# uthree/tinyvc

Measured on AMD Instinct MI355X. Metric: audio-samples/sec (16 kHz) end-to-end VC, higher is better.
Workload: dtype f32 (fp32 in / out / accumulate; channel contractions as two-term fp16 splits on v_mfma_f32_32x32x16_f16: 22-bit significands, three part-products per fp32 product)

## Files before the change

tinyvc_amd/csrc/filter_up24s.hip:

```cpp
#include "conv_s2.h"
#include "small_kernels.h"
#include "split_fp16.h"
#include "tvc_common.h"

namespace tvc {

typedef unsigned u32x2 __attribute__((ext_vector_type(2)));
typedef float f32x4s __attribute__((ext_vector_type(4)));

constexpr int U24S_WPE = 2;

template <int W_, int D1_, int D2_, bool SECOND_, int E_>
struct U24S {
    static constexpr int C = 24, W = W_, D1 = D1_, D2 = D2_, E = E_, H = D1_ + D2_;
    static constexpr bool SECOND = SECOND_;
    static constexpr int NWAVES = 8, NT = 64 * NWAVES;
    static constexpr int W2 = W + 2 * E;
    static constexpr int NT2 = (W2 + 31) / 32, W2r = NT2 * 32;
    static constexpr int NT1 = (W2 + 2 * D2 + 31) / 32;
    static constexpr int HP = NT1 * 32;
    static constexpr int XW = W2 + 2 * H;
    static constexpr int XP = XW;
    static constexpr int PS = W2r + 16;
    static constexpr int ITEMS = 3 * XW, XPER = (ITEMS + NT - 1) / NT;
    static constexpr int PIECES = Up24sBlob::PIECES, FL = 320;
    static constexpr int LDS_BYTES = (6 * XP + 6 * HP + PIECES * 64) * 16 + (FL + C * PS) * 4;
    static_assert(NT2 <= NWAVES, "one second-conv tile per wave");
    static_assert(XW - H >= W2, "residual columns");
    static_assert(LDS_BYTES <= 160 * 1024, "LDS");
};

struct Up24SArgs {
    const float* x;
    const uint4* cond;
    float cbw, cbb;
    float* out;
    const u32x4* img;
    int len, xf, tiles_per_utt, ntiles;
    float interp_scale;
    const float* amax_x;
    const float* amax_c;
    float* amax_y;
    RagDev rag;
};

__device__ __forceinline__ void split4(const float (&v)[4], u32x2& p1, u32x2& p2) {
#pragma unroll
    for (int j = 0; j < 2; ++j) {
        unsigned q1, q2;
        split2(v[2 * j], v[2 * j + 1], q1, q2);
        p1[j] = q1;
        p2[j] = q2;
    }
}

__device__ __forceinline__ void ld8_g8(float (&dst)[8], const float* base, unsigned byte_off) {
    const uint4* b4 = reinterpret_cast<const uint4*>(base);
    const f32x4s q0 = __builtin_bit_cast(f32x4s, ldg_so4(b4, byte_off)), q1 = __builtin_bit_cast(f32x4s, ldg_so4(b4, byte_off + 16u));
    dst[0] = q0.x; dst[1] = q0.y; dst[2] = q0.z; dst[3] = q0.w;
    dst[4] = q1.x; dst[5] = q1.y; dst[6] = q1.z; dst[7] = q1.w;
}

template <int P, int DIL>
__device__ __forceinline__ void conv24_phase(f32x16& hi, f32x16& lo, const u32x4* src, const u32x4* wt, int col, int lo_c, int hi_c, int lane) {
    const int lh = lane >> 5;
    constexpr int TAP0[5] = {0, 0, 1, 2, 2}, GRP0[5] = {0, 2, 1, 0, 2};
    constexpr int TAP1[5] = {0, 1, 1, 2, 2}, GRP1[5] = {1, 0, 2, 1, 2};
    int row[5];
#pragma unroll
    for (int s = 0; s < 5; ++s) {
        int c = col + (lh ? TAP1[s] : TAP0[s]) * DIL;
        c = c < lo_c ? lo_c : (c > hi_c ? hi_c : c);
        row[s] = (lh ? GRP1[s] : GRP0[s]) * P + c;
    }
    f16x8 af[2][2], bf[2][2];
    auto frags = [&](int s, int fb) __attribute__((always_inline)) {
#pragma unroll
        for (int p = 0; p < 2; ++p) {
            bf[fb][p] = __builtin_bit_cast(f16x8, src[p * 3 * P + row[s]]);
            af[fb][p] = __builtin_bit_cast(f16x8, wt[(s * 2 + p) * 64 + lane]);
        }
    };
    frags(0, 0);
#pragma unroll
    for (int s = 0; s < 5; ++s) {
        const int fb = s & 1;
        if (s + 1 < 5) frags(s + 1, fb ^ 1);
        __builtin_amdgcn_sched_barrier(0);
        lo = TVC_MFMA16(af[fb][1], bf[fb][0], lo);
        hi = TVC_MFMA16(af[fb][0], bf[fb][0], hi);
        lo = TVC_MFMA16(af[fb][0], bf[fb][1], lo);
        __builtin_amdgcn_sched_barrier(0);
    }
}

template <class CF, bool RAG>
__global__ __launch_bounds__(CF::NT) __attribute__((amdgpu_waves_per_eu(U24S_WPE))) void up24s_kernel(Up24SArgs a) {
    constexpr int C = CF::C, W = CF::W, D1 = CF::D1, D2 = CF::D2, H = CF::H, E = CF::E, NT = CF::NT;
    constexpr int XP = CF::XP, HP = CF::HP, PS = CF::PS, XW = CF::XW, XPER = CF::XPER;
    extern __shared__ __attribute__((aligned(16))) uint4 smem_u[];
    u32x4* Xs = reinterpret_cast<u32x4*>(smem_u);
    u32x4* Hs = Xs + 6 * XP;
    u32x4* Wt = Hs + 6 * HP;
    float* Fl = reinterpret_cast<float*>(Wt + CF::PIECES * 64);
    float* R = Fl + CF::FL;
    const int tid = threadIdx.x, lane = tid & 63, wave = tid >> 6;
    const int l31 = lane & 31, lh = lane >> 5;
    const int rs = a.len;
    const int rsl = CF::SECOND ? rs : rs / a.xf;
    int bh = 0;
    auto utt = [&](int tile) __attribute__((always_inline)) { return rag_tile<RAG>(a.rag, tile, a.tiles_per_utt, rs, bh).b; };

    for (int i = tid; i < CF::PIECES * 64 + Up24sBlob::FLOATS / 4; i += NT) Wt[i] = a.img[i];

    float xr0[XPER][8], xr1[XPER][8], lam[XPER];
    int ig8[XPER], ic[XPER];
    bool ilive[XPER];
#pragma unroll
    for (int i = 0; i < XPER; ++i) {
        const int idx = tid + i * NT;
        int g = idx / XW;
        ic[i] = idx - g * XW;
        ilive[i] = idx < CF::ITEMS;
        ig8[i] = 8 * (g > 2 ? 2 : g);
    }
    auto fetch = [&](int tile) __attribute__((always_inline)) {
        const RagTile rt = rag_tile<RAG>(a.rag, tile, a.tiles_per_utt, rs, bh);
        const int len = rt.len, lin = CF::SECOND ? len : len / a.xf;
        const int px0 = rt.tin * W - E - H;
        const uint4* xb = reinterpret_cast<const uint4*>(RAG ? a.x + 8L * (CF::SECOND ? rt.off : rt.off / a.xf) : a.x + (long)rt.b * C * rsl);
        auto ld8 = [&](float (&dst)[8], unsigned o) __attribute__((always_inline)) {
            const f32x4s q0 = __builtin_bit_cast(f32x4s, ldg_so4(xb, o)), q1 = __builtin_bit_cast(f32x4s, ldg_so4(xb, o + 16u));
            dst[0] = q0.x; dst[1] = q0.y; dst[2] = q0.z; dst[3] = q0.w;
            dst[4] = q1.x; dst[5] = q1.y; dst[6] = q1.z; dst[7] = q1.w;
        };
#pragma unroll
        for (int i = 0; i < XPER; ++i) {
            int p = px0 + ic[i];
            p = p < 0 ? 0 : (p > len - 1 ? len - 1 : p);
            const int g = ig8[i] >> 3;
            if (CF::SECOND) {
                ld8(xr0[i], 32u * (unsigned)(g * rsl + p));
            } else {
                const Lerp lc = lerp_coord(p, a.interp_scale, lin);
                lam[i] = lc.w1;
                ld8(xr0[i], 32u * (unsigned)(g * rsl + lc.i0));
                ld8(xr1[i], 32u * (unsigned)(g * rsl + lc.i1));
            }
        }
    };
    auto deposit = [&](float xs) __attribute__((always_inline)) {
#pragma unroll
        for (int i = 0; i < XPER; ++i) {
            if (!ilive[i]) continue;
            const int g = ig8[i] >> 3, c = ic[i];
            float v[8];
            if (CF::SECOND) {
#pragma unroll
                for (int j = 0; j < 8; ++j) v[j] = xr0[i][j];
            } else {
                const float w0 = 1.f - lam[i];
#pragma unroll
                for (int j = 0; j < 8; ++j) v[j] = fmaf(w0, xr0[i][j], __fmul_rn(lam[i], xr1[i][j]));
            }
            const int rc = c - H;
            if (rc >= 0 && rc < CF::W2r) {
#pragma unroll
                for (int j = 0; j < 8; ++j) R[(ig8[i] + j) * PS + rc] = v[j];
            }
#pragma unroll
            for (int j = 0; j < 8; ++j) v[j] = fmaxf(v[j], 0.1f * v[j]) * xs;
            uint4 p1, p2;
            split8(v, p1, p2);
            Xs[(0 + g) * XP + c] = __builtin_bit_cast(u32x4, p1);
            Xs[(3 + g) * XP + c] = __builtin_bit_cast(u32x4, p2);
        }
    };

    int tile, tend;
    tile_range(a.ntiles, tile, tend);
    if (tile < tend) {
        bh = utt(tile);
        fetch(tile);
        deposit(bfp_load_u(a.amax_x, bh).s);
    }
    slab_barrier();
    const float wsa = Fl[Up24sBlob::SA], wsb = Fl[Up24sBlob::SB], wssc = Fl[Up24sBlob::SSC], wssh = Fl[Up24sBlob::SSH], wl1 = Fl[Up24sBlob::L1A], bamax = Fl[Up24sBlob::BMA];
    float mx_run = 0.f;
    int mx_b = bh;
    int slot_b = -1;
    Bfp sx{1.f, 1.f}, sc{1.f, 1.f}, sh_{1.f, 1.f};

    for (; tile < tend; ++tile) {
        const RagTile rt = rag_tile<RAG>(a.rag, tile, a.tiles_per_utt, rs, bh);
        const int b = rt.b, len = rt.len;
        bh = b;
        if (!CF::SECOND && a.amax_y && b != mx_b) {
            amax_flush_wg(a.amax_y + mx_b, mx_run, Fl + Up24sBlob::FLOATS);
            mx_run = 0.f;
            mx_b = b;
        }
        if (b != slot_b) {
            slot_b = b;
            const float slot_x = a.amax_x ? sload_f32(a.amax_x + b) : 0.f;
            const float slot_c = a.amax_c ? sload_f32(a.amax_c + b) : 0.f;
            sx = a.amax_x ? bfp_from_amax(slot_x) : Bfp{1.f, 1.f};
            sc = a.amax_c ? norm_from_amax(fmaf(a.cbw, slot_c, a.cbb)) : Bfp{1.f, 1.f};
            sh_ = a.amax_x ? bfp_from_amax(fmaf(wl1, slot_x, bamax)) : Bfp{1.f, 1.f};
        }
        const int t0 = rt.tin * W;
        const int ph0 = t0 - E - D2;
        const int p20 = t0 - E;
        const int next = tile + 1;

        float keep[3][4];
        bool keep_live = false;
        unsigned keep_oo = 0;
        float wv_out = 0.f;
        bool wv_live = false;
        int wv_off = 0;
        u32x4 cq[2][2];
        if (wave < CF::NT2) {
            const uint4* cb = RAG ? a.cond + rt.off : a.cond + (long)b * 6 * rs;
            int t = p20 + wave * 32 + l31;
            t = t < 0 ? 0 : (t > len - 1 ? len - 1 : t);
            const unsigned o0 = 16u * (unsigned)(lh * rs + t), o1 = 16u * (unsigned)t;
#pragma unroll
            for (int p = 0; p < 2; ++p) {
                cq[0][p] = ldg_so4(cb + (long)(3 * p) * rs, o0);
                cq[1][p] = ldg_so4(cb + (long)(3 * p + 2) * rs, o1);
            }
        }

        bool fetched = false;
        for (int nt = wave; nt < CF::NT1; nt += CF::NWAVES) {
            f32x16 acc, alo;
#pragma unroll
            for (int r = 0; r < 16; ++r) acc[r] = alo[r] = 0.f;
            const int h = nt * 32 + l31;
            conv24_phase<XP, D1>(acc, alo, Xs, Wt, h, 0, XW - 1, lane);
            if (!fetched) {
                fetched = true;
                if (next < tend) fetch(next);
            }
            const float c = wsa * sx.inv, cl = c * kLoInv;
#pragma unroll
            for (int g = 0; g < 3; ++g) {
                const f32x4s bv = *reinterpret_cast<const f32x4s*>(Fl + Up24sBlob::BA + 8 * g + 4 * lh);
                float v[4];
#pragma unroll
                for (int q = 0; q < 4; ++q) {
                    const float t = comb(acc[4 * g + q], alo[4 * g + q], c, cl) + bv[q];
                    v[q] = fmaxf(t, 0.1f * t) * sh_.s;
                }
                u32x2 p1, p2;
                split4(v, p1, p2);
                const auto qx = __builtin_amdgcn_permlane32_swap(p1[0], p2[0], false, false);
                const auto qy = __builtin_amdgcn_permlane32_swap(p1[1], p2[1], false, false);
                const u32x4 row = {qx[0], qy[0], qx[1], qy[1]};
                *reinterpret_cast<u32x4*>(Hs + (3 * lh + g) * HP + h) = row;
            }
        }
        if (!fetched && next < tend) fetch(next);
        slab_barrier();

        if (wave < CF::NT2) {
            const int n = wave * 32 + l31;
            const int t = p20 + n;
            f16x8 cf[2][2];
            {
                const u32x4 z = {0u, 0u, 0u, 0u};
#pragma unroll
                for (int p = 0; p < 2; ++p) {
                    cf[0][p] = __builtin_bit_cast(f16x8, cq[0][p]);
                    cf[1][p] = __builtin_bit_cast(f16x8, lh ? z : cq[1][p]);
                }
            }
            const float cb = wsb * sh_.inv, cbl = cb * kLoInv, c1 = wssc * sc.inv, c1l = c1 * kLoInv, c2 = wssh * sc.inv, c2l = c2 * kLoInv;
            float hv[3][4];
            {
                f32x16 acc, alo;
#pragma unroll
                for (int r = 0; r < 16; ++r) acc[r] = alo[r] = 0.f;
                const int lo = -ph0 > 0 ? -ph0 : 0;
                const int hi = (len - 1 - ph0) < (HP - 1) ? (len - 1 - ph0) : (HP - 1);
                conv24_phase<HP, D2>(acc, alo, Hs, Wt + 10 * 64, n, lo, hi, lane);
#pragma unroll
                for (int g = 0; g < 3; ++g) {
                    const f32x4s bb = *reinterpret_cast<const f32x4s*>(Fl + Up24sBlob::BB + 8 * g + 4 * lh);
#pragma unroll
                    for (int q = 0; q < 4; ++q) hv[g][q] = comb(acc[4 * g + q], alo[4 * g + q], cb, cbl) + bb[q];
                }
            }
            __builtin_amdgcn_sched_barrier(0);
            f32x16 asc, lsc, ash, lsh;
#pragma unroll
            for (int r = 0; r < 16; ++r) asc[r] = lsc[r] = ash[r] = lsh[r] = 0.f;
#pragma unroll
            for (int s = 0; s < 2; ++s) {
                f16x8 fa[2][2];
#pragma unroll
                for (int mt = 0; mt < 2; ++mt)
#pragma unroll
                    for (int p = 0; p < 2; ++p) fa[mt][p] = __builtin_bit_cast(f16x8, Wt[(20 + (s * 2 + mt) * 2 + p) * 64 + lane]);
                lsc = TVC_MFMA16(fa[0][1], cf[s][0], lsc);
                lsh = TVC_MFMA16(fa[1][1], cf[s][0], lsh);
                asc = TVC_MFMA16(fa[0][0], cf[s][0], asc);
                ash = TVC_MFMA16(fa[1][0], cf[s][0], ash);
                lsc = TVC_MFMA16(fa[0][0], cf[s][1], lsc);
                lsh = TVC_MFMA16(fa[1][0], cf[s][1], lsh);
            }
            float mx = 0.f;
#pragma unroll
            for (int g = 0; g < 3; ++g) {
                float v4[4];
                const f32x4s bs = *reinterpret_cast<const f32x4s*>(Fl + Up24sBlob::BSC + 8 * g + 4 * lh);
                const f32x4s bh = *reinterpret_cast<const f32x4s*>(Fl + Up24sBlob::BSH + 8 * g + 4 * lh);
#pragma unroll
                for (int q = 0; q < 4; ++q) {
                    const int m = 8 * g + 4 * lh + q;
                    const float hval = hv[g][q];
                    const float scv = comb(asc[4 * g + q], lsc[4 * g + q], c1, c1l) + bs[q];
                    const float shv = comb(ash[4 * g + q], lsh[4 * g + q], c2, c2l) + bh[q];
                    const float res = R[m * PS + n];
                    const float v = __fadd_rn(__fadd_rn(__fmul_rn(hval, scv), shv), res);
                    v4[q] = v;
                    if (CF::SECOND) R[m * PS + n] = v;
                }
                if (!CF::SECOND) {
#pragma unroll
                    for (int q = 0; q < 4; ++q) keep[g][q] = v4[q];
                    if (n < W && t < len) mx = fmaxf(mx, fmaxf(fmaxf(fabsf(v4[0]), fabsf(v4[1])), fmaxf(fabsf(v4[2]), fabsf(v4[3]))));
                }
            }
            mx_run = fmaxf(mx_run, mx);
            keep_live = !CF::SECOND && n < W && t < len;
            keep_oo = 32u * (unsigned)t + 16u * (unsigned)lh;
        }
        if (CF::SECOND) {
            slab_barrier();
            const float* W7 = Fl + Up24sBlob::W75;
            const int part = tid & 7;
            const int lo = -p20 > 0 ? -p20 : 0;
            const int hi = (len - 1 - p20) < (CF::W2 - 1) ? (len - 1 - p20) : (CF::W2 - 1);
            const bool interior = lo == 0 && hi == CF::W2 - 1;
            for (int g0 = 0; g0 < (W + 3) / 4; g0 += NT / 8) {
                const int g = g0 + (tid >> 3);
                float o4[4] = {0.f, 0.f, 0.f, 0.f};
                if (4 * g < W) {
#pragma unroll
                    for (int cc = 0; cc < 3; ++cc) {
                        const int c = part * 3 + cc;
                        float xv[10], wv[7];
                        if (E == 3 && interior) {
                            const f32x4s* rp = reinterpret_cast<const f32x4s*>(R + c * PS + 4 * g);
                            const f32x4s r0 = rp[0], r1 = rp[1], r2 = rp[2];
                            xv[0] = r0[0]; xv[1] = r0[1]; xv[2] = r0[2]; xv[3] = r0[3];
                            xv[4] = r1[0]; xv[5] = r1[1]; xv[6] = r1[2]; xv[7] = r1[3];
                            xv[8] = r2[0]; xv[9] = r2[1];
                        } else {
#pragma unroll
                            for (int i = 0; i < 10; ++i) {
                                int col = 4 * g + E - 3 + i;
                                col = col < lo ? lo : (col > hi ? hi : col);
                                xv[i] = R[c * PS + col];
                            }
                        }
#pragma unroll
                        for (int j = 0; j < 7; ++j) wv[j] = W7[c * 7 + j];
#pragma unroll
                        for (int q = 0; q < 4; ++q)
#pragma unroll
                            for (int j = 0; j < 7; ++j) o4[q] = fmaf(wv[j], xv[q + j], o4[q]);
                    }
                }
#pragma unroll
                for (int q = 0; q < 4; ++q) {
                    o4[q] += __shfl_xor(o4[q], 1);
                    o4[q] += __shfl_xor(o4[q], 2);
                    o4[q] += __shfl_xor(o4[q], 4);
                }
                const int o = 4 * g + part;
                const float v = part == 0 ? o4[0] : (part == 1 ? o4[1] : (part == 2 ? o4[2] : o4[3]));
                static_assert((W + 3) / 4 <= NT / 8, "one output per thread: it waits in a register until the deposit is through");
                wv_out = v + Fl[Up24sBlob::B75];
                wv_live = part < 4 && o < W && t0 + o < len;
                wv_off = t0 + o;
            }
        }
        slab_barrier();
        if (next < tend) {
            const int bn = utt(next);
            deposit(bn == slot_b ? sx.s : bfp_load_u(a.amax_x, bn).s);
        }
        if (CF::SECOND) {
            float* wrow = RAG ? a.out + (long)a.rag.row[b] * a.rag.Tmax * kHop : a.out + (long)b * rs;
            if (wv_live) wrow[wv_off] = wv_out;
        } else if (keep_live) {
            float* ob = RAG ? a.out + 8L * rt.off : a.out + (long)b * C * rs;
#pragma unroll
            for (int g = 0; g < 3; ++g) stg_so4(ob + (long)g * 8 * rs, keep_oo, keep[g]);
        }
        slab_barrier();
    }
    if (!CF::SECOND && a.amax_y && tend > (int)((long)a.ntiles * blockIdx.x / gridDim.x)) amax_flush_wg(a.amax_y + mx_b, mx_run, Fl + Up24sBlob::FLOATS);
}

template <class CF>
static int launch_up24s(tvc_ctx* ctx, hipStream_t s, Up24SArgs a, int B) {
    const size_t lds = (size_t)CF::LDS_BYTES;
    TVC_CHECK((lds_optin<up24s_kernel<CF, false>, up24s_kernel<CF, true>>(ctx, (int)lds, "up24s")));
    a.tiles_per_utt = (a.len + CF::W - 1) / CF::W;
    a.ntiles = a.tiles_per_utt * B;
    TVC_CHECK(rag_tiles(ctx, s, B, a.len, CF::W, &a.rag, &a.ntiles, "up24s", kHop));
    const int grid = a.ntiles < ctx->ncu ? a.ntiles : ctx->ncu;
    if (ctx->rag) hipLaunchKernelGGL((up24s_kernel<CF, true>), dim3(grid), dim3(CF::NT), lds, s, a);
    else hipLaunchKernelGGL((up24s_kernel<CF, false>), dim3(grid), dim3(CF::NT), lds, s, a);
    return launch_check(ctx, "up24s");
}

constexpr int U24S_WA = 250, U24S_WB = 250;

int run_up24_split(tvc_ctx* ctx, hipStream_t s, const UpW& u, const float* x, const float* cond_planes, float cbw, float cbb, float* x1, float* wave, int B, int len,
                   const float* amax_x, const float* amax_c, float* amax_x1) {
    if (!u.s24a || !u.s24b) return fail(ctx, TVC_ERR_STATE, "up24s: the split weight blobs of the 24-channel block are missing");
    if ((long)len * 24 * 4 >= (1L << 32)) return fail(ctx, TVC_ERR_ARG, "up24s: utterance too long for 32-bit element offsets");
    using CA = U24S<U24S_WA, 1, 3, false, 0>;
    using CB = U24S<U24S_WB, 9, 27, true, 3>;
    Up24SArgs a{};
    a.len = len;
    a.xf = u.factor;
    a.interp_scale = (float)(1.0 / (double)u.factor);
    a.cond = reinterpret_cast<const uint4*>(cond_planes);
    a.cbw = cbw;
    a.cbb = cbb;
    a.amax_c = amax_c;
    a.x = x;
    a.amax_x = amax_x;
    a.out = x1;
    a.amax_y = amax_x1;
    a.img = reinterpret_cast<const u32x4*>(u.s24a);
    TVC_CHECK(launch_up24s<CA>(ctx, s, a, B));
    a.x = x1;
    a.amax_x = amax_x1;
    a.out = wave;
    a.amax_y = nullptr;
    a.img = reinterpret_cast<const u32x4*>(u.s24b);
    return launch_up24s<CB>(ctx, s, a, B);
}

struct Down0SArgs {
    const float* source;
    const float* energy;
    float* out;
    uint4* planes;
    float* y2;
    const u32x4* img;
    int len, tiles_per_utt, ntiles;
    const float* amax_x;
    float* amax_y;
    RagDev rag;
};

template <bool RAG>
static __global__ __launch_bounds__(512) __attribute__((amdgpu_waves_per_eu(4))) void down0s_kernel(Down0SArgs a) {
    constexpr int W = 254, XW = 256, XP = XW, NT = 512;
    extern __shared__ __attribute__((aligned(16))) uint4 smem_d[];
    u32x4* Xs = reinterpret_cast<u32x4*>(smem_d);
    u32x4* Wt = Xs + 2 * 6 * XP;
    float* Bi = reinterpret_cast<float*>(Wt + Down0sBlob::PIECES * 64);
    const int tid = threadIdx.x, lane = tid & 63, wave = tid >> 6;
    const int l31 = lane & 31, lh = lane >> 5;
    const int rs = a.len;
    for (int i = tid; i < Down0sBlob::PIECES * 64 + Down0sBlob::FLOATS / 4; i += NT) Wt[i] = a.img[i];

    const int g = tid >> 8, c = tid & 255;
    float xa[8], xe = 0.f;
// ... 421 lines not shown
```

tinyvc_amd/csrc/pack.hip:

```cpp
#include <algorithm>
#include <cmath>

#include "tvc_common.h"

namespace tvc {

size_t ArenaBuilder::put(const float** slot, const float* v, size_t n) {
    const size_t off = (buf.size() + 63) & ~size_t(63);
    buf.resize(off + n, 0.f);
    std::copy(v, v + n, buf.begin() + off);
    fix.push_back({slot, off});
    return off;
}

namespace {

int pad_m(int M) {
    if (M <= 32) return 32;
    if (M <= 64) return 64;
    if (M <= 96) return 96;
    if (M % 96 == 0 && M % 128 != 0) return M;
    return (M + 127) / 128 * 128;
}

// ... 163 lines not shown
        a6(pb, Ab, 0, sa);
        ab.fix.push_back({&pb->wjoint, off_a});
    }
    size_t a6(PackedW* pw, const std::vector<float>& At, int group_rows, const std::vector<float>& scale) {
        const int taps = pw->taps, cin = pw->cin, nslab = ((cin + 15) / 16 + 5) / 6 * 6;
        const int MT = image_mt(pw, group_rows);
        std::vector<float> img((size_t)nslab * taps * MT * 2 * 256, 0.f);
        uint16_t* o = reinterpret_cast<uint16_t*>(img.data());
        for (int s = 0; s < nslab; ++s)
            for (int tap = 0; tap < taps; ++tap)
                for (int mt = 0; mt < MT; ++mt)
                    for (int lane = 0; lane < 64; ++lane)
                        for (int j = 0; j < 8; ++j) {
                            const int ci = s * 16 + 8 * (lane >> 5) + j, m = image_row(pw, group_rows, mt * 32 + (lane & 31));
                            const float w = (ci < cin && m < pw->M) ? At[(size_t)(ci * taps + tap) * pw->Mpad + m] : 0.f;
                            const size_t base = (((size_t)(s * taps + tap) * MT + mt) * 2 * 64 + lane) * 8 + j;
                            split2(w, scale[mt], &o[base], &o[base + 512]);
                        }
        pw->MT6 = MT;
        pw->S6 = nslab;
        const size_t off = ab.put(&pw->A6, img);
        ab.put(&pw->wscale, scale);
        host_wscale[pw] = scale;
        return off;
    }
    void film_u(FilmU* fu, const std::string& conv_name, const std::string& film, int C, const std::string& first_conv) {
        const size_t CC = (size_t)C * C;
        const float* w = get(conv_name + ".weight", 3 * CC);
        const float* b = get(conv_name + ".bias", C);
        const float* wsc = get(film + ".to_scale.weight", CC);
        const float* bsc = get(film + ".to_scale.bias", C);
        const float* wsh = get(film + ".to_shift.weight", CC);
        const float* bsh = get(film + ".to_shift.bias", C);
        if (!w || !b || !wsc || !bsc || !wsh || !bsh) return;
        const int MT = C / 32, nslab = C / 16, mblocks = C / 96;
        auto tile_scale = [&](const float* wt, int per_row, int mt) { return pow2_scale(amax(wt + (size_t)mt * 32 * per_row, (size_t)32 * per_row)) * (1.f / 8192.f); };
        std::vector<float> tab((size_t)6 * C);
        auto row = [&](int r) { return &tab[(size_t)r * C]; };
        float *scale_conv = row(FilmU::TAB_SCALE), *scale_sc = row(FilmU::TAB_SSC), *scale_sh = row(FilmU::TAB_SSH);
        std::copy(b, b + C, row(FilmU::TAB_BIAS));
        std::copy(bsc, bsc + C, row(FilmU::TAB_BSC));
        std::copy(bsh, bsh + C, row(FilmU::TAB_BSH));
        for (int mt = 0; mt < MT; ++mt) {
            std::fill_n(scale_conv + 32 * mt, 32, tile_scale(w, 3 * C, mt));
            std::fill_n(scale_sc + 32 * mt, 32, tile_scale(wsc, C, mt));
            std::fill_n(scale_sh + 32 * mt, 32, tile_scale(wsh, C, mt));
        }
        std::vector<float> img((size_t)mblocks * nslab * 30 * 64 * 4, 0.f);
        uint16_t* o = reinterpret_cast<uint16_t*>(img.data());
        for (int mb = 0; mb < mblocks; ++mb)
            for (int s = 0; s < nslab; ++s)
                for (int q = 0; q < 30; ++q) {
                    const bool conv = q < 18;
                    const int qq = conv ? q : q - 18, grp = qq / 6, mi = (qq % 6) / 2, part = qq % 2, mt = mb * 3 + mi;
                    for (int lane = 0; lane < 64; ++lane)
                        for (int j = 0; j < 8; ++j) {
                            const int m = mt * 32 + (lane & 31), ci = s * 16 + 8 * (lane >> 5) + j;
                            float x;
                            if (conv) x = w[((size_t)m * C + ci) * 3 + grp] / scale_conv[m];
                            else if (grp == 0) x = wsc[(size_t)m * C + ci] / scale_sc[m];
                            else x = wsh[(size_t)m * C + ci] / scale_sh[m];
                            const uint16_t h1 = f16_bits(x);
                            o[((((size_t)mb * nslab + s) * 30 + q) * 64 + lane) * 8 + j] = part == 0 ? h1 : f16_bits(x - f16_value(h1));
                        }
                }
        bound(first_conv, C, 3 * C, &fu->hb_w, &fu->hb_b);
        fu->C = C;
        ab.put(&fu->img, img);
        ab.put(&fu->tab, tab);
    }
    void up24s_half(const float** slot, const std::string& ca, const std::string& cb, const std::string& film, const std::string& c5,
                    const std::string& out7) {
        using L = Up24sBlob;
        constexpr int C = 24;
        const float* wa = get(ca + ".weight", C * C * 3);
        const float* ba = get(ca + ".bias", C);
        const float* wb = get(cb + ".weight", C * C * 3);
        const float* bb = get(cb + ".bias", C);
        const float* wsc = get(film + ".to_scale.weight", C * C);
        const float* bsc = get(film + ".to_scale.bias", C);
        const float* wsh = get(film + ".to_shift.weight", C * C);
        const float* bsh = get(film + ".to_shift.bias", C);
        if (!wa || !ba || !wb || !bb || !wsc || !bsc || !wsh || !bsh) return;
        std::vector<float> img(L::PIECES * 256 + L::FLOATS, 0.f);
        float* fl = img.data() + L::PIECES * 256;
        fl[L::SA] = pow2_scale(amax(wa, C * C * 3));
        fl[L::SB] = pow2_scale(amax(wb, C * C * 3));
        fl[L::SSC] = pow2_scale(amax(wsc, C * C));
        fl[L::SSH] = pow2_scale(amax(wsh, C * C));
        put_k24(img, 0, 2, wa, C, C, 3, &fl[L::SA]);
        put_k24(img, 10, 2, wb, C, C, 3, &fl[L::SB]);
        put_k24(img, 20, 4, wsc, C, C, 1, &fl[L::SSC]);
        put_k24(img, 22, 4, wsh, C, C, 1, &fl[L::SSH]);
        std::copy(ba, ba + C, fl + L::BA);
        std::copy(bb, bb + C, fl + L::BB);
        std::copy(bsc, bsc + C, fl + L::BSC);
        std::copy(bsh, bsh + C, fl + L::BSH);
        const RowL1 r = row_l1(wa, ba, C, C * 3);
        fl[L::L1A] = (float)(r.w * 1.0000002);
        fl[L::BMA] = (float)r.b;
        if (!c5.empty()) {
            const float* w5 = get(c5 + ".weight", C * C);
            const float* b5 = get(c5 + ".bias", C);
            const float* w7 = get(out7 + ".weight", C * 7);
            const float* b7 = get(out7 + ".bias", 1);
            if (!w5 || !b5 || !w7 || !b7) return;
            double bias = b7[0];
            for (int c = 0; c < C; ++c)
                for (int j = 0; j < 7; ++j) {
                    double acc = 0.0;
                    for (int m = 0; m < C; ++m) acc += (double)w7[(size_t)m * 7 + j] * (double)w5[(size_t)m * C + c];
                    fl[L::W75 + c * 7 + j] = (float)acc;
                }
            for (int m = 0; m < C; ++m)
                for (int j = 0; j < 7; ++j) bias += (double)w7[(size_t)m * 7 + j] * (double)b5[m];
            fl[L::B75] = (float)bias;
        }
        ab.put(slot, img);
    }
    void down0s(const float** slot, const std::string& name, float* bound_w, float* bound_b) {
        using L = Down0sBlob;
        constexpr int C = 24, CI = 17;
        const float* w = get(name + ".weight", C * CI * 3);
        const float* b = get(name + ".bias", C);
        if (!w || !b) return;
        std::vector<float> img(L::PIECES * 256 + L::FLOATS, 0.f);
        float* fl = img.data() + L::PIECES * 256;
        fl[L::SCALE] = pow2_scale(amax(w, C * CI * 3));
        put_k24(img, 0, 2, w, C, CI, 3, &fl[L::SCALE]);
        std::copy(b, b + C, fl + L::BIAS);
        const RowL1 r = row_l1(w, b, C, CI * 3);
        fl[L::BW] = *bound_w = (float)(r.w * 1.0001);
        fl[L::BB] = *bound_b = (float)r.b * 1.0001f;
        ab.put(slot, img);
    }
    void conv24s(const float** slot, const std::string& name, int M, const std::string& extra_bias = "", const PackedW* joint = nullptr) {
        constexpr int CI = 24;
        const int MT = (M + 31) / 32;
        const float* w = get(name + ".weight", (size_t)M * CI * 3);
        const float* b = get(name + ".bias", M);
        const float* eb = extra_bias.empty() ? nullptr : get(extra_bias, M);
        if (!w || !b || (!extra_bias.empty() && !eb)) return;
        std::vector<float> img((size_t)K24_PIECES * MT * 256 + Conv24sBlob::FLOATS, 0.f);
        float* fl = img.data() + (size_t)K24_PIECES * MT * 256;
        float* sc = fl + Conv24sBlob::SCALE;
        if (joint) {
            auto it = host_wscale.find(joint);
            if (it == host_wscale.end() || (int)it->second.size() != MT) return note(name + " (its joint image is not packed yet)");
            std::copy(it->second.begin(), it->second.end(), sc);
        } else {
            for (int mt = 0; mt < MT; ++mt) sc[mt] = pow2_scale(amax(w + (size_t)32 * mt * CI * 3, (size_t)(std::min(M, 32 * mt + 32) - 32 * mt) * CI * 3));
        }
        put_k24(img, 0, 2 * MT, w, M, CI, 3, sc);
        for (int m = 0; m < M; ++m) fl[Conv24sBlob::BIAS + m] = b[m] + (eb ? eb[m] : 0.f);
        ab.put(slot, img);
    }
    void convnext(const std::string& p, ConvNeXtW* w, int C, int dil) {
        w->C = C;
        w->dilation = dil;
        raw(p + ".c1.weight", &w->dw_w, (size_t)C * 7);
        raw(p + ".c1.bias", &w->dw_b, C);
        const float* g = get(p + ".norm.gamma", C);
        const float* bt = get(p + ".norm.beta", C);
        if (g) ab.put(&w->ln_g, g, C);
        if (bt) ab.put(&w->ln_b, bt, C);
        if (g && bt) {
            const RowL1 r = row_l1(g, bt, C, 1);
            w->ln_bound = std::sqrt((float)C) * (float)r.w + (float)r.b;
        }
        conv({p + ".c2"}, &w->c2, C, 1);
        raw(p + ".grn.gamma", &w->grn_g, 2 * C);
        raw(p + ".grn.beta", &w->grn_b, 2 * C);
        conv({p + ".c3"}, &w->c3, 2 * C, 1);
        const float* w3 = get(p + ".c3.weight", (size_t)C * 2 * C);
        const float* b3 = get(p + ".c3.bias", C);
        const float* gb = get(p + ".grn.beta", 2 * C);
        if (w3 && b3 && gb) {
            std::vector<float> fb(w->c3.Mpad, 0.f);
            for (int m = 0; m < C; ++m) {
                double acc = b3[m];
                for (int k = 0; k < 2 * C; ++k) acc += (double)w3[(size_t)m * 2 * C + k] * (double)gb[k];
                fb[m] = (float)acc;
            }
            ab.put(&w->c3_bias_grn, fb);
        }
    }
};

}

void pack_constants(tvc_ctx* ctx, ArenaBuilder* ab) {
    const int N = kNfft;
    const double two_pi = 6.283185307179586476925286766559;
    std::vector<float> t960(2 * 960), t1920(2 * 961 + 2), hann(N);
    for (int j = 0; j < 960; ++j) {
        t960[2 * j] = (float)std::cos(two_pi * j / 960.0);
        t960[2 * j + 1] = (float)std::sin(two_pi * j / 960.0);
    }
    for (int k = 0; k <= 960; ++k) {
// ... 111 lines not shown
```

tinyvc_amd/csrc/tvc_common.h:

```cpp
#pragma once
#include <hip/hip_runtime.h>

#include <atomic>
#include <cstdarg>
#include <cstdint>
#include <cstdio>
#include <cstring>
#include <map>
#include <string>
#include <vector>

#include "../../include/tinyvc_hip.h"
#include "ragged.h"

namespace tvc {

constexpr int kSampleRate = 24000;
constexpr int kNfft = 1920;
constexpr int kHop = 480;
constexpr int kBins = 961;
constexpr int kSslDim = 768;
constexpr int kSslCh = 384;
constexpr int kPitchCh = 128;
constexpr int kPitchClasses = 512;
constexpr int kSrcCh = 128;
constexpr int kHarm = 15;
constexpr int kSolaCross = 1920, kSolaSearch = 1920, kSolaDelay = 3840;
constexpr int kSolaGroups = 8, kSolaPartFloats = 16384;

struct PackedW {
    const float* bias = nullptr;
    const float* A6 = nullptr;
    const float* wscale = nullptr;
    const float* wjoint = nullptr;
    int M = 0, K = 0, Mpad = 0, Kpad = 0, cin = 0, taps = 1, MT6 = 0, S6 = 0;
};

struct ConvNeXtW {
    const float* dw_w = nullptr;
    const float* dw_b = nullptr;
    const float* ln_g = nullptr;
    const float* ln_b = nullptr;
    PackedW c2, c3;
    const float* grn_g = nullptr;
    const float* grn_b = nullptr;
    const float* c3_bias_grn = nullptr;
    float ln_bound = 0.f;
    int C = 0, dilation = 1;
};

constexpr int K24_PIECES = 10;
struct Up24sBlob {
    static constexpr int PIECES = 28;
    static constexpr int BA = 0, BB = 32, BSC = 64, BSH = 96;
    static constexpr int W75 = 128, B75 = 296;
    static constexpr int SA = 297, SB = 298, SSC = 299, SSH = 300;
    static constexpr int L1A = 301, BMA = 302;
    static constexpr int FLOATS = 304;
};
struct Down0sBlob {
    static constexpr int PIECES = K24_PIECES;
    static constexpr int BIAS = 0;
    static constexpr int BW = 29, BB = 30;
    static constexpr int SCALE = 31;
    static constexpr int FLOATS = 32;
};
struct Conv24sBlob {
    static constexpr int BIAS = 0;
    static constexpr int SCALE = 62;
    static constexpr int FLOATS = 64;
};

struct DownW {
    PackedW res, c1, c2, c3;
    const float* c3res_bias = nullptr;
    const float* s24c1 = nullptr;
    const float* s24c2 = nullptr;
    const float* s24c3r = nullptr;
    float b1_w = 0.f, b1_b = 0.f, b2_w = 0.f, b2_b = 0.f;
    int cin = 0, cout = 0, factor = 1;
};
struct FilmU {
    static constexpr int TAB_BIAS = 0, TAB_SCALE = 1, TAB_BSC = 2, TAB_BSH = 3, TAB_SSC = 4, TAB_SSH = 5;
    const float* img = nullptr;
    const float* tab = nullptr;
    int C = 0;
    float hb_w = 0.f, hb_b = 0.f;
};
struct UpW {
    PackedW c1, c2, c3, c4, c5, film1, film2;
    FilmU fu1, fu2;
    const float* s24a = nullptr;
    const float* s24b = nullptr;
    float c5_bw = 0.f, c5_bb = 0.f;
    int cin = 0, cout = 0, factor = 1;
};

struct HostTensor {
    std::vector<float> data;
    std::vector<int64_t> shape;
};

struct ArenaBuilder {
    std::vector<float> buf;
    std::vector<std::pair<const float**, size_t>> fix;
    size_t put(const float** slot, const float* v, size_t n);
    size_t put(const float** slot, const std::vector<float>& v) { return put(slot, v.data(), v.size()); }
    void resolve(const float* arena) const {
        for (auto& f : fix) *f.first = arena + f.second;
    }
};

}

struct tvc_prof_region {
    std::string name;
    hipEvent_t a = nullptr, b = nullptr;
};

struct tvc_ctx {
    int device = 0;
    int ncu = 0;
    int profiling = 0;
    std::vector<tvc_prof_region> regions;
    std::vector<hipEvent_t> event_pool;
    hipStream_t side = nullptr;
    hipEvent_t ev_fork = nullptr, ev_join = nullptr;
    hipEvent_t ev_fork2 = nullptr, ev_join2 = nullptr, ev_amps = nullptr;
    tvc::RagHost* rag = nullptr;
    int rag_batch_frames = 0;
    bool enc_ready = false, dec_ready = false;
    char enc_missing[160] = {0}, dec_missing[160] = {0};
    std::map<std::string, tvc::HostTensor> host;
    std::vector<float> pitch_table;
    float* arena = nullptr;
    float* const_arena = nullptr;
    size_t arena_floats = 0;
    char err[512] = {0};

    const float* fft_tw960 = nullptr;
// ... 230 lines not shown
```

Measured before the change: 718.5 million.

## Slide up24s window as LDS ring and fold final 7-tap conv into MFMA

In the second up24s stage, consecutive tiles of the same utterance now reuse the overlapping halo columns of the input, hidden and residual LDS buffers as ring buffers. Only the new W columns are fetched and only the new hidden columns are recomputed, instead of reloading and recomputing the whole window. The fused 1x1+7-tap output convolution moves from a per-thread scalar FMA loop over the residual buffer to an in-register MFMA contraction (24→7 channels) stored into a small Y buffer, followed by a 7-term diagonal sum. This adds ring-index wrapping, extra LDS and a new fp16-split packed weight, and changes rounding in the output head.

```diff
diff --git a/tinyvc_amd/csrc/filter_up24s.hip b/tinyvc_amd/csrc/filter_up24s.hip
--- a/tinyvc_amd/csrc/filter_up24s.hip
+++ b/tinyvc_amd/csrc/filter_up24s.hip
@@ -21,10 +21,17 @@
     static constexpr int HP = NT1 * 32;
     static constexpr int XW = W2 + 2 * H;
     static constexpr int XP = XW;
+    static constexpr bool RING = SECOND;
+    static constexpr int SX0 = XW - W;
+    static constexpr int SH0 = W2 + 2 * D2 - NWAVES * 32;
     static constexpr int PS = W2r + 16;
+    static constexpr int YS = W2r + 8;
     static constexpr int ITEMS = 3 * XW, XPER = (ITEMS + NT - 1) / NT;
-    static constexpr int PIECES = Up24sBlob::PIECES, FL = 320;
-    static constexpr int LDS_BYTES = (6 * XP + 6 * HP + PIECES * 64) * 16 + (FL + C * PS) * 4;
+    static constexpr int PIECES = SECOND ? Up24sBlob::PIECES2 : Up24sBlob::PIECES, FL = 320;
+    static constexpr int RW = RING ? XW - H : W2r, RS = RING ? 304 : PS;
+    static constexpr int LDS_BYTES = (6 * XP + 6 * HP + PIECES * 64) * 16 + (FL + C * RS + (SECOND ? 7 * YS : 0)) * 4;
+    static_assert(!RING || (SH0 >= 0 && SH0 <= W2 + 2 * D2 - W && SH0 + NWAVES * 32 - 1 + 2 * D1 < XW), "the slide's first-conv round covers the new Hs columns from Xs columns of this window");
+    static_assert(!RING || (HP >= W2 + 2 * D2 && RS >= RW && SX0 >= H && W <= XP && W <= HP && W <= RS), "ring capacities");
     static_assert(NT2 <= NWAVES, "one second-conv tile per wave");
     static_assert(XW - H >= W2, "residual columns");
     static_assert(LDS_BYTES <= 160 * 1024, "LDS");
@@ -61,8 +68,13 @@
     dst[4] = q1.x; dst[5] = q1.y; dst[6] = q1.z; dst[7] = q1.w;
 }
 
-template <int P, int DIL>
-__device__ __forceinline__ void conv24_phase(f32x16& hi, f32x16& lo, const u32x4* src, const u32x4* wt, int col, int lo_c, int hi_c, int lane) {
+__device__ __forceinline__ int ring_wrap(int i, int cap) {
+    const unsigned u = (unsigned)i, w = u - (unsigned)cap;
+    return (int)(u < w ? u : w);
+}
+
+template <int P, int DIL, bool RING = false>
+__device__ __forceinline__ void conv24_phase(f32x16& hi, f32x16& lo, const u32x4* src, const u32x4* wt, int col, int lo_c, int hi_c, int lane, int org = 0) {
     const int lh = lane >> 5;
     constexpr int TAP0[5] = {0, 0, 1, 2, 2}, GRP0[5] = {0, 2, 1, 0, 2};
     constexpr int TAP1[5] = {0, 1, 1, 2, 2}, GRP1[5] = {1, 0, 2, 1, 2};
@@ -71,6 +83,7 @@
     for (int s = 0; s < 5; ++s) {
         int c = col + (lh ? TAP1[s] : TAP0[s]) * DIL;
         c = c < lo_c ? lo_c : (c > hi_c ? hi_c : c);
+        if (RING) c = ring_wrap(c + org, P);
         row[s] = (lh ? GRP1[s] : GRP0[s]) * P + c;
     }
     f16x8 af[2][2], bf[2][2];
@@ -97,13 +110,15 @@
 template <class CF, bool RAG>
 __global__ __launch_bounds__(CF::NT) __attribute__((amdgpu_waves_per_eu(U24S_WPE))) void up24s_kernel(Up24SArgs a) {
     constexpr int C = CF::C, W = CF::W, D1 = CF::D1, D2 = CF::D2, H = CF::H, E = CF::E, NT = CF::NT;
-    constexpr int XP = CF::XP, HP = CF::HP, PS = CF::PS, XW = CF::XW, XPER = CF::XPER;
+    constexpr int XP = CF::XP, HP = CF::HP, PS = CF::PS, RS = CF::RS, XW = CF::XW, XPER = CF::XPER;
+    constexpr bool RING = CF::RING;
     extern __shared__ __attribute__((aligned(16))) uint4 smem_u[];
     u32x4* Xs = reinterpret_cast<u32x4*>(smem_u);
     u32x4* Hs = Xs + 6 * XP;
     u32x4* Wt = Hs + 6 * HP;
     float* Fl = reinterpret_cast<float*>(Wt + CF::PIECES * 64);
     float* R = Fl + CF::FL;
+    float* Y = R + C * RS;
     const int tid = threadIdx.x, lane = tid & 63, wave = tid >> 6;
     const int l31 = lane & 31, lh = lane >> 5;
     const int rs = a.len;
@@ -124,7 +139,19 @@
         ilive[i] = idx < CF::ITEMS;
         ig8[i] = 8 * (g > 2 ? 2 : g);
     }
-    auto fetch = [&](int tile) __attribute__((always_inline)) {
+    int sg8[XPER], sc_[XPER];
+    bool slive[XPER];
+    if (RING) {
+#pragma unroll
+        for (int i = 0; i < XPER; ++i) {
+            const int idx = tid + i * NT;
+            int g = idx / W;
+            sc_[i] = CF::SX0 + idx - g * W;
+            slive[i] = idx < 3 * W;
+            sg8[i] = 8 * (g > 2 ? 2 : g);
+        }
+    }
+    auto fetch = [&](int tile, bool slide) __attribute__((always_inline)) {
         const RagTile rt = rag_tile<RAG>(a.rag, tile, a.tiles_per_utt, rs, bh);
         const int len = rt.len, lin = CF::SECOND ? len : len / a.xf;
         const int px0 = rt.tin * W - E - H;
@@ -136,9 +163,9 @@
         };
 #pragma unroll
         for (int i = 0; i < XPER; ++i) {
-            int p = px0 + ic[i];
+            int p = px0 + (RING && slide ? sc_[i] : ic[i]);
             p = p < 0 ? 0 : (p > len - 1 ? len - 1 : p);
-            const int g = ig8[i] >> 3;
+            const int g = (RING && slide ? sg8[i] : ig8[i]) >> 3;
             if (CF::SECOND) {
                 ld8(xr0[i], 32u * (unsigned)(g * rsl + p));
             } else {
@@ -149,11 +176,11 @@
             }
         }
     };
-    auto deposit = [&](float xs) __attribute__((always_inline)) {
+    auto deposit = [&](float xs, bool slide, int ox, int orr) __attribute__((always_inline)) {
 #pragma unroll
         for (int i = 0; i < XPER; ++i) {
-            if (!ilive[i]) continue;
-            const int g = ig8[i] >> 3, c = ic[i];
+            if (!(RING && slide ? slive[i] : ilive[i])) continue;
+            const int g8 = RING && slide ? sg8[i] : ig8[i], g = g8 >> 3, c = RING && slide ? sc_[i] : ic[i];
             float v[8];
             if (CF::SECOND) {
 #pragma unroll
@@ -164,16 +191,18 @@
                 for (int j = 0; j < 8; ++j) v[j] = fmaf(w0, xr0[i][j], __fmul_rn(lam[i], xr1[i][j]));
             }
             const int rc = c - H;
-            if (rc >= 0 && rc < CF::W2r) {
-#pragma unroll
-                for (int j = 0; j < 8; ++j) R[(ig8[i] + j) * PS + rc] = v[j];
+            if (rc >= 0 && rc < CF::RW) {
+                const int rr = RING ? ring_wrap(orr + rc, RS) : rc;
+#pragma unroll
+                for (int j = 0; j < 8; ++j) R[(g8 + j) * RS + rr] = v[j];
             }
 #pragma unroll
             for (int j = 0; j < 8; ++j) v[j] = fmaxf(v[j], 0.1f * v[j]) * xs;
             uint4 p1, p2;
             split8(v, p1, p2);
-            Xs[(0 + g) * XP + c] = __builtin_bit_cast(u32x4, p1);
-            Xs[(3 + g) * XP + c] = __builtin_bit_cast(u32x4, p2);
+            const int cx = RING ? ring_wrap(ox + c, XP) : c;
+            Xs[(0 + g) * XP + cx] = __builtin_bit_cast(u32x4, p1);
+            Xs[(3 + g) * XP + cx] = __builtin_bit_cast(u32x4, p2);
         }
     };
 
@@ -181,8 +210,8 @@
     tile_range(a.ntiles, tile, tend);
     if (tile < tend) {
         bh = utt(tile);
-        fetch(tile);
-        deposit(bfp_load_u(a.amax_x, bh).s);
+        fetch(tile, false);
+        deposit(bfp_load_u(a.amax_x, bh).s, false, 0, 0);
     }
     slab_barrier();
     const float wsa = Fl[Up24sBlob::SA], wsb = Fl[Up24sBlob::SB], wssc = Fl[Up24sBlob::SSC], wssh = Fl[Up24sBlob::SSH], wl1 = Fl[Up24sBlob::L1A], bamax = Fl[Up24sBlob::BMA];
@@ -190,6 +219,8 @@
     int mx_b = bh;
     int slot_b = -1;
     Bfp sx{1.f, 1.f}, sc{1.f, 1.f}, sh_{1.f, 1.f};
+    bool slid = false;
+    int ox = 0, oh = 0, orr = 0;
 
     for (; tile < tend; ++tile) {
         const RagTile rt = rag_tile<RAG>(a.rag, tile, a.tiles_per_utt, rs, bh);
@@ -212,6 +243,8 @@
         const int ph0 = t0 - E - D2;
         const int p20 = t0 - E;
         const int next = tile + 1;
+        const int bn = next < tend ? utt(next) : -1;
+        const bool slide_next = RING && bn == b;
 
         float keep[3][4];
         bool keep_live = false;
@@ -233,15 +266,16 @@
         }
 
         bool fetched = false;
-        for (int nt = wave; nt < CF::NT1; nt += CF::NWAVES) {
+        const int nt1 = RING && slid ? CF::NWAVES : CF::NT1, h0 = RING && slid ? CF::SH0 : 0;
+        for (int nt = wave; nt < nt1; nt += CF::NWAVES) {
             f32x16 acc, alo;
 #pragma unroll
             for (int r = 0; r < 16; ++r) acc[r] = alo[r] = 0.f;
-            const int h = nt * 32 + l31;
-            conv24_phase<XP, D1>(acc, alo, Xs, Wt, h, 0, XW - 1, lane);
+            const int h = h0 + nt * 32 + l31;
+            conv24_phase<XP, D1, RING>(acc, alo, Xs, Wt, h, 0, XW - 1, lane, ox);
             if (!fetched) {
                 fetched = true;
-                if (next < tend) fetch(next);
+                if (next < tend) fetch(next, slide_next);
             }
             const float c = wsa * sx.inv, cl = c * kLoInv;
 #pragma unroll
@@ -258,10 +292,10 @@
                 const auto qx = __builtin_amdgcn_permlane32_swap(p1[0], p2[0], false, false);
                 const auto qy = __builtin_amdgcn_permlane32_swap(p1[1], p2[1], false, false);
                 const u32x4 row = {qx[0], qy[0], qx[1], qy[1]};
-                *reinterpret_cast<u32x4*>(Hs + (3 * lh + g) * HP + h) = row;
-            }
-        }
-        if (!fetched && next < tend) fetch(next);
+                *reinterpret_cast<u32x4*>(Hs + (3 * lh + g) * HP + (RING ? ring_wrap(oh + h, HP) : h)) = row;
+            }
+        }
+        if (!fetched && next < tend) fetch(next, slide_next);
         slab_barrier();
 
         if (wave < CF::NT2) {
@@ -284,7 +318,7 @@
                 for (int r = 0; r < 16; ++r) acc[r] = alo[r] = 0.f;
                 const int lo = -ph0 > 0 ? -ph0 : 0;
                 const int hi = (len - 1 - ph0) < (HP - 1) ? (len - 1 - ph0) : (HP - 1);
-                conv24_phase<HP, D2>(acc, alo, Hs, Wt + 10 * 64, n, lo, hi, lane);
+                conv24_phase<HP, D2, RING>(acc, alo, Hs, Wt + 10 * 64, n, lo, hi, lane, oh);
 #pragma unroll
                 for (int g = 0; g < 3; ++g) {
                     const f32x4s bb = *reinterpret_cast<const f32x4s*>(Fl + Up24sBlob::BB + 8 * g + 4 * lh);
@@ -311,6 +345,7 @@
                 lsh = TVC_MFMA16(fa[1][0], cf[s][1], lsh);
             }
             float mx = 0.f;
+            const int nr = RING ? ring_wrap(orr + n, RS) : n;
 #pragma unroll
             for (int g = 0; g < 3; ++g) {
                 float v4[4];
@@ -322,10 +357,13 @@
                     const float hval = hv[g][q];
                     const float scv = comb(asc[4 * g + q], lsc[4 * g + q], c1, c1l) + bs[q];
                     const float shv = comb(ash[4 * g + q], lsh[4 * g + q], c2, c2l) + bh[q];
-                    const float res = R[m * PS + n];
+                    const float res = R[m * RS + nr];
                     const float v = __fadd_rn(__fadd_rn(__fmul_rn(hval, scv), shv), res);
                     v4[q] = v;
-                    if (CF::SECOND) R[m * PS + n] = v;
+                }
+                if (CF::SECOND) {
+#pragma unroll
+                    for (int q = 0; q < 4; ++q) keep[g][q] = v4[q];
                 }
                 if (!CF::SECOND) {
 #pragma unroll
@@ -336,63 +374,70 @@
             mx_run = fmaxf(mx_run, mx);
             keep_live = !CF::SECOND && n < W && t < len;
             keep_oo = 32u * (unsigned)t + 16u * (unsigned)lh;
+            if (CF::SECOND) {
+                __builtin_amdgcn_sched_barrier(0);
+                float m2 = 0.f;
+#pragma unroll
+                for (int g = 0; g < 3; ++g)
+#pragma unroll
+                    for (int q = 0; q < 4; ++q) m2 = fmaxf(m2, fabsf(keep[g][q]));
+                const Bfp s2 = bfp_from_amax(wave_max(m2));
+                u32x2 p[2][3];
+#pragma unroll
+                for (int g = 0; g < 3; ++g) {
+                    const float v[4] = {keep[g][0] * s2.s, keep[g][1] * s2.s, keep[g][2] * s2.s, keep[g][3] * s2.s};
+                    split4(v, p[0][g], p[1][g]);
+                }
+                f16x8 xf[2][2];
+#pragma unroll
+                for (int pt = 0; pt < 2; ++pt) {
+                    const auto e0 = __builtin_amdgcn_permlane32_swap(p[pt][0][0], p[pt][1][0], false, false);
+                    const auto e1 = __builtin_amdgcn_permlane32_swap(p[pt][0][1], p[pt][1][1], false, false);
+                    const auto f0 = __builtin_amdgcn_permlane32_swap(p[pt][2][0], 0u, false, false);
+                    const auto f1 = __builtin_amdgcn_permlane32_swap(p[pt][2][1], 0u, false, false);
+                    xf[0][pt] = __builtin_bit_cast(f16x8, u32x4{e0[0], e1[0], e0[1], e1[1]});
+                    xf[1][pt] = __builtin_bit_cast(f16x8, u32x4{f0[0], f1[0], f0[1], f1[1]});
+                }
+                f32x16 yh, yl;
+#pragma unroll
+                for (int r = 0; r < 16; ++r) yh[r] = yl[r] = 0.f;
+#pragma unroll
+                for (int s = 0; s < 2; ++s) {
+                    const f16x8 w1 = __builtin_bit_cast(f16x8, Wt[(Up24sBlob::P75 + 2 * s) * 64 + lane]), w2 = __builtin_bit_cast(f16x8, Wt[(Up24sBlob::P75 + 2 * s + 1) * 64 + lane]);
+                    yl = TVC_MFMA16(w2, xf[s][0], yl);
+                    yh = TVC_MFMA16(w1, xf[s][0], yh);
+                    yl = TVC_MFMA16(w1, xf[s][1], yl);
+                }
+                const float c7 = Fl[Up24sBlob::S75] * s2.inv, c7l = c7 * kLoInv;
+#pragma unroll
+                for (int q = 0; q < 4; ++q)
+                    if (4 * lh + q < 7) Y[(4 * lh + q) * CF::YS + n] = comb(yh[q], yl[q], c7, c7l);
+            }
         }
         if (CF::SECOND) {
             slab_barrier();
-            const float* W7 = Fl + Up24sBlob::W75;
-            const int part = tid & 7;
             const int lo = -p20 > 0 ? -p20 : 0;
             const int hi = (len - 1 - p20) < (CF::W2 - 1) ? (len - 1 - p20) : (CF::W2 - 1);
-            const bool interior = lo == 0 && hi == CF::W2 - 1;
-            for (int g0 = 0; g0 < (W + 3) / 4; g0 += NT / 8) {
-                const int g = g0 + (tid >> 3);
-                float o4[4] = {0.f, 0.f, 0.f, 0.f};
-                if (4 * g < W) {
-#pragma unroll
-                    for (int cc = 0; cc < 3; ++cc) {
-                        const int c = part * 3 + cc;
-                        float xv[10], wv[7];
-                        if (E == 3 && interior) {
-                            const f32x4s* rp = reinterpret_cast<const f32x4s*>(R + c * PS + 4 * g);
-                            const f32x4s r0 = rp[0], r1 = rp[1], r2 = rp[2];
-                            xv[0] = r0[0]; xv[1] = r0[1]; xv[2] = r0[2]; xv[3] = r0[3];
-                            xv[4] = r1[0]; xv[5] = r1[1]; xv[6] = r1[2]; xv[7] = r1[3];
-                            xv[8] = r2[0]; xv[9] = r2[1];
-                        } else {
-#pragma unroll
-                            for (int i = 0; i < 10; ++i) {
-                                int col = 4 * g + E - 3 + i;
-                                col = col < lo ? lo : (col > hi ? hi : col);
-                                xv[i] = R[c * PS + col];
-                            }
-                        }
-#pragma unroll
-                        for (int j = 0; j < 7; ++j) wv[j] = W7[c * 7 + j];
-#pragma unroll
-                        for (int q = 0; q < 4; ++q)
-#pragma unroll
-                            for (int j = 0; j < 7; ++j) o4[q] = fmaf(wv[j], xv[q + j], o4[q]);
-                    }
-                }
-#pragma unroll
-                for (int q = 0; q < 4; ++q) {
-                    o4[q] += __shfl_xor(o4[q], 1);
-                    o4[q] += __shfl_xor(o4[q], 2);
-                    o4[q] += __shfl_xor(o4[q], 4);
-                }
-                const int o = 4 * g + part;
-                const float v = part == 0 ? o4[0] : (part == 1 ? o4[1] : (part == 2 ? o4[2] : o4[3]));
-                static_assert((W + 3) / 4 <= NT / 8, "one output per thread: it waits in a register until the deposit is through");
-                wv_out = v + Fl[Up24sBlob::B75];
-                wv_live = part < 4 && o < W && t0 + o < len;
-                wv_off = t0 + o;
-            }
+            static_assert(W <= NT, "one output per thread: it waits in a register until the deposit is through");
+            float acc = Fl[Up24sBlob::B75];
+#pragma unroll
+            for (int j = 0; j < 7; ++j) {
+                int col = tid + j + E - 3;
+                col = col < lo ? lo : (col > hi ? hi : col);
+                acc = __fadd_rn(acc, Y[j * CF::YS + col]);
+            }
+            wv_out = acc;
+            wv_live = tid < W && t0 + tid < len;
+            wv_off = t0 + tid;
         }
         slab_barrier();
-        if (next < tend) {
-            const int bn = utt(next);
-            deposit(bn == slot_b ? sx.s : bfp_load_u(a.amax_x, bn).s);
-        }
+        if (RING) {
+            ox = slide_next ? ring_wrap(ox + W, XP) : 0;
+            oh = slide_next ? ring_wrap(oh + W, HP) : 0;
+            orr = slide_next ? ring_wrap(orr + W, RS) : 0;
+            slid = slide_next;
+        }
+        if (next < tend) deposit(bn == slot_b ? sx.s : bfp_load_u(a.amax_x, bn).s, slide_next, ox, orr);
         if (CF::SECOND) {
             float* wrow = RAG ? a.out + (long)a.rag.row[b] * a.rag.Tmax * kHop : a.out + (long)b * rs;
             if (wv_live) wrow[wv_off] = wv_out;
diff --git a/tinyvc_amd/csrc/pack.hip b/tinyvc_amd/csrc/pack.hip
--- a/tinyvc_amd/csrc/pack.hip
+++ b/tinyvc_amd/csrc/pack.hip
@@ -269,8 +269,9 @@
         const float* wsh = get(film + ".to_shift.weight", C * C);
         const float* bsh = get(film + ".to_shift.bias", C);
         if (!wa || !ba || !wb || !bb || !wsc || !bsc || !wsh || !bsh) return;
-        std::vector<float> img(L::PIECES * 256 + L::FLOATS, 0.f);
-        float* fl = img.data() + L::PIECES * 256;
+        const int pieces = c5.empty() ? L::PIECES : L::PIECES2;
+        std::vector<float> img(pieces * 256 + L::FLOATS, 0.f);
+        float* fl = img.data() + pieces * 256;
         fl[L::SA] = pow2_scale(amax(wa, C * C * 3));
         fl[L::SB] = pow2_scale(amax(wb, C * C * 3));
         fl[L::SSC] = pow2_scale(amax(wsc, C * C));
@@ -302,6 +303,11 @@
             for (int m = 0; m < C; ++m)
                 for (int j = 0; j < 7; ++j) bias += (double)w7[(size_t)m * 7 + j] * (double)b5[m];
             fl[L::B75] = (float)bias;
+            float w75t[7 * C];
+            for (int c = 0; c < C; ++c)
+                for (int j = 0; j < 7; ++j) w75t[j * C + c] = fl[L::W75 + c * 7 + j];
+            fl[L::S75] = pow2_scale(amax(w75t, 7 * C));
+            put_k24(img, L::P75, 2, w75t, 7, C, 1, &fl[L::S75]);
         }
         ab.put(slot, img);
     }
diff --git a/tinyvc_amd/csrc/tvc_common.h b/tinyvc_amd/csrc/tvc_common.h
--- a/tinyvc_amd/csrc/tvc_common.h
+++ b/tinyvc_amd/csrc/tvc_common.h
@@ -52,10 +52,12 @@
 constexpr int K24_PIECES = 10;
 struct Up24sBlob {
     static constexpr int PIECES = 28;
+    static constexpr int P75 = 28, PIECES2 = 32;
     static constexpr int BA = 0, BB = 32, BSC = 64, BSH = 96;
     static constexpr int W75 = 128, B75 = 296;
     static constexpr int SA = 297, SB = 298, SSC = 299, SSH = 300;
     static constexpr int L1A = 301, BMA = 302;
+    static constexpr int S75 = 303;
     static constexpr int FLOATS = 304;
 };
 struct Down0sBlob {
```

Result: no change. 722.4 million (median of 6 runs) (+0.5%).
